# livesense-inc/fanlin-rs

Measured on AMD Instinct MI355X. Metric: images/sec whole-node (1080p→300×200 resize+encode); p50 per-image ms, higher is better.
Workload: dtype u8 (exact, as f16 subnormals) x the reference's f32 weights as three f16 terms -> f32 sums (vertical, v_mfma_f32_16x16x32_f16); 24-bit fixed-point intermediate (2^-14 steps, three i8 planes) x 24-bit fixed-point weights (2^-24 steps, three i8 digits), eight of the nine digit products -> exact i32 (h

## Files before the change

### fanlin-rs_amd/csrc/fl_batch.cpp

```cpp
#include <stdio.h>
#include <stdlib.h>

#include <algorithm>
#include <cassert>
#include <memory>
#include <optional>

#include "fl_context.h"

using namespace fl;

namespace {


enum Stage1Kind { S1_NONE = 0, S1_PLACE = 1, S1_GENERIC = 2, S1_STREAM = 3, S1_NEAREST = 4, S1_MFMA = 5, S1_TILE = 6, S1_WTILE = 7 };
constexpr size_t kNoScratch = ~(size_t)0;

struct Work {
    flgpu_plan plan;
    const flgpu_params *p;
    uint32_t cs, pre, sw, sh;
    Stage1Kind s1;
    const uint8_t *src;
    uint8_t *s1_dst = nullptr;
// ... 155 lines not shown
            if (!R) uniform = false;
            else {
                for (uint32_t r = 0; r < R; ++r)
                    for (uint32_t t = 0; t < T; ++t) {
                        const auto &v = by_job[jobs_in_order[r * T + t]];
                        for (uint32_t s2 = 0; s2 < S; ++s2) per_wg[triples[t][s2]].push_back(v[s2]);
                    }
                const uint32_t Lp = P - R * T;
                if (Lp) {
                    const uint32_t nt = (uint32_t)plan->tiles.size();
                    const uint32_t nb = std::max(1u, std::min(nt, (2u * G + Lp * S - 1u) / (Lp * S)));
                    const std::vector<MfmaItem> &bands = plan->items_for(nb);
                    std::vector<MfmaItem> units;
                    for (uint32_t p2 = R * T; p2 < P; ++p2)
                        for (MfmaItem u : bands) { u.job = jobs_in_order[p2]; units.push_back(u); }
                    std::stable_sort(units.begin(), units.end(), [](const MfmaItem &x, const MfmaItem &y) { return x.kb1 - x.kb0 > y.kb1 - y.kb0; });
                    std::vector<uint64_t> load(G, 0);
                    for (uint32_t b = 0; b < G; ++b) for (const MfmaItem &a : per_wg[b]) load[b] += a.kb1 - a.kb0;
                    for (const MfmaItem &u : units) {
                        uint32_t best = 0;
                        for (uint32_t b = 1; b < G; ++b) if (load[b] < load[best]) best = b;
                        per_wg[best].push_back(u);
                        load[best] += u.kb1 - u.kb0 + 2u;
                    }
                }
            }
        }
    }
    if (!uniform) { for (auto &v : per_wg) v.clear(); classic(); }
    std::vector<MfmaItem> flat;
    lists.assign(2u * G, 0u);
    for (uint32_t b = 0; b < G; ++b) {
        lists[2 * b] = (uint32_t)flat.size();
        lists[2 * b + 1] = (uint32_t)per_wg[b].size();
        flat.insert(flat.end(), per_wg[b].begin(), per_wg[b].end());
    }
    mitems.resize(base);
    mitems.insert(mitems.end(), flat.begin(), flat.end());
    nitems = (uint32_t)flat.size();
}

void fill_job(const Work &w, Job &j)
{
    memset(&j, 0, sizeof(j));
    const flgpu_plan &pl = w.plan;
    j.src = w.src;
    j.dst = w.s1_dst;
    j.src_bytes = w.sw * w.sh * w.cs;
    j.sw = w.sw; j.sh = w.sh;
    j.rw = pl.resized_w; j.rh = pl.resized_h;
    j.cx = pl.crop_x; j.cy = pl.crop_y;
    if (pl.letterboxed) {
        j.cw = std::min(pl.resized_w - pl.crop_x, pl.out_w - pl.place_x);
        j.ch = std::min(pl.resized_h - pl.crop_y, pl.out_h - pl.place_y);
    } else {
        j.cw = pl.out_w; j.ch = pl.out_h;
    }
    j.dw = pl.out_w; j.dh = pl.out_h;
    j.ox = pl.place_x; j.oy = pl.place_y;
    if (w.luma_mid) { j.dw = j.cw; j.dh = j.ch; j.ox = 0; j.oy = 0; }
    j.fill = (uint32_t)w.p->fill_r | ((uint32_t)w.p->fill_g << 8) | ((uint32_t)w.p->fill_b << 16) | (255u << 24);
    j.vtab = w.vtab; j.htab = w.htab;
    j.pad1 = w.tile_w;
    j.pad0 = w.tile_vplan;
    if (w.s1 == S1_NEAREST) {
        const float ry = (float)w.sh / (float)pl.resized_h, rx = (float)w.sw / (float)pl.resized_w;
        memcpy(&j.vtab, &ry, 4); memcpy(&j.htab, &rx, 4);
    }
}


uint32_t tile_width_for(const HostAxis &h, const HostAxis &v, uint32_t cx, uint32_t cw, uint32_t cy, uint32_t ch, uint32_t mc)
{
    for (uint32_t y0 = cy; y0 < cy + ch; y0 += 8u) {
        const uint32_t y1 = std::min(y0 + 8u, cy + ch);
        if (v.left[y1 - 1] + v.count[y1 - 1] - v.left[y0] > kTileVRows) return 0;
    }
    const uint32_t nc_max = kTileLdsFloats / (8u * mc);
    for (uint32_t tw = 256; tw >= 16; tw >>= 1) {
        bool fits = true;
        for (uint32_t x0 = cx; x0 < cx + cw && fits; x0 += tw) {
            const uint32_t x1 = std::min(x0 + tw, cx + cw);
            if (h.left[x1 - 1] + h.count[x1 - 1] - h.left[x0] > nc_max) fits = false;
            if (h.woff[x1 - 1] + h.count[x1 - 1] - h.woff[x0] > kTileWeightFloats) fits = false;
        }
        if (fits) return tw;
    }
    return 0;
}

void build_tile_vplan(const HostAxis &v, uint32_t cy, uint32_t ch, std::vector<uint32_t> &blk)
{
    const uint32_t nb = (ch + 7u) / 8u;
    uint32_t stride = 1;
    for (uint32_t b = 0; b < nb; ++b) {
        const uint32_t y0 = cy + 8u * b, y1 = std::min(y0 + 8u, cy + ch);
        stride = std::max(stride, v.left[y1 - 1] + v.count[y1 - 1] - v.left[y0]);
    }
    TileVPlanHeader hd{nb, stride, (uint32_t)(sizeof(TileVPlanHeader) / 4), (uint32_t)(sizeof(TileVPlanHeader) / 4) + 2u * nb};
    blk.assign((size_t)hd.dense_off + (size_t)nb * stride * 8u, 0u);
    memcpy(blk.data(), &hd, sizeof(hd));
    for (uint32_t b = 0; b < nb; ++b) {
        const uint32_t y0 = cy + 8u * b, y1 = std::min(y0 + 8u, cy + ch);
        const uint32_t top = v.left[y0], rv = v.left[y1 - 1] + v.count[y1 - 1] - top;
        blk[hd.bands_off + 2u * b] = top;
        blk[hd.bands_off + 2u * b + 1u] = rv;
        float *dense = reinterpret_cast<float *>(blk.data() + hd.dense_off) + (size_t)b * stride * 8u;
        for (uint32_t oy = y0; oy < y1; ++oy)
            for (uint32_t k = 0; k < v.count[oy]; ++k) dense[(size_t)(v.left[oy] + k - top) * 8u + (oy - y0)] = v.weights[v.woff[oy] + k];
    }
}

template <class Item, class Len>
void xcd_interleave(Item *first, uint32_t nitems, Len len_of)
{
#ifdef FL_EXPERIMENT
    static const bool no_xcd_order = [] { const char *e = getenv("FLGPU_NO_XCD_ORDER"); return e && e[0] == '1'; }();
#else
    constexpr bool no_xcd_order = false;
#endif
    std::vector<Item> tmp;
    for (uint32_t a = 0; a < nitems && !no_xcd_order;) {
        uint32_t b = a;
        const uint32_t len = len_of(first[a]);
        while (b < nitems && len_of(first[b]) == len) ++b;
        for (uint32_t g0 = a; g0 < b;) {
            uint32_t g1 = g0, njob = 0, prev = 0xffffffffu, per = 0, cur = 0;
            bool uniform = true;
            while (g1 < b) {
                if (first[g1].job != prev) {
                    if (njob == 8) break;
                    if (njob >= 1) { if (per == 0) per = cur; else if (cur != per) uniform = false; }
                    ++njob; prev = first[g1].job; cur = 0;
                }
                ++cur; ++g1;
            }
            if (per == 0) per = cur; else if (cur != per) uniform = false;
            if (uniform && njob > 1 && per > 1) {
                tmp.assign(first + g0, first + g1);
                for (uint32_t s2 = 0; s2 < per; ++s2)
                    for (uint32_t j2 = 0; j2 < njob; ++j2) first[g0 + s2 * njob + j2] = tmp[j2 * per + s2];
            }
            g0 = g1;
        }
        a = b;
    }
}



int jpeg_scratch(const flgpu_plan &pl, ScratchSizes &s)
{
    if (pl.out_w > 65535u || pl.out_h > 65535u) return FLGPU_ERR_UNSUPPORTED;
    const size_t units = (size_t)(pl.plane_w / 8u) * (pl.plane_h / 8u) * 3u;
    if (units * kJpegMaxUnitBytes * 8 >= ((size_t)1 << 32)) return FLGPU_ERR_UNSUPPORTED;
    s.jpeg_coef += align_up(units * sizeof(JpegUnit), 256);
    s.jpeg_off += align_up((units + 1) * sizeof(uint32_t), 256);
    s.jpeg_raw += align_up(units * kAcWordsPerUnit * sizeof(uint32_t), 256);
    return FLGPU_OK;
}

int png_scratch(const flgpu_plan &pl, ScratchSizes &s)
{
    const uint64_t fb = png_filtered_bytes(pl.out_w, pl.out_h, pl.out_c);
    if ((uint64_t)s.png_rows + pl.out_h >= (1ull << 31) || (uint64_t)s.png_segs + png_segments(fb) >= (1ull << 31)) return FLGPU_ERR_UNSUPPORTED;
    s.png_filt += align_up(fb, 256);
    s.png_rows += pl.out_h;
    s.png_segs += (uint32_t)png_segments(fb);
    return FLGPU_OK;
}

int webpll_scratch(const flgpu_plan &pl, ScratchSizes &s)
{
    const uint64_t npix = (uint64_t)pl.out_w * pl.out_h;
    if ((uint64_t)s.wll_tiles + webpll_tiles(npix) >= (1ull << 31) || webpll_max_out_bytes(pl.out_w, pl.out_h) / 4u >= (1ull << 32))
        return FLGPU_ERR_UNSUPPORTED;
    s.wll_res += align_up(npix * 4u, 256);
    s.wll_tok += align_up(npix * 2u, 256);
    s.wll_stream += align_up(webpll_max_out_bytes(pl.out_w, pl.out_h), 256);
    s.wll_tiles += (uint32_t)webpll_tiles(npix);
    s.wll_pics++;
    return FLGPU_OK;
}

bool vp8_fe_lf(uint32_t fe) { return fe >= FLGPU_FE_WEBP_LOSSY_LF && fe <= FLGPU_FE_WEBP_LOSSY_I4_AP_LF; }
bool vp8_fe_i4(uint32_t fe) { return fe == FLGPU_FE_WEBP_LOSSY_I4 || fe == FLGPU_FE_WEBP_LOSSY_I4_AP || fe == FLGPU_FE_WEBP_LOSSY_I4_LF || fe == FLGPU_FE_WEBP_LOSSY_I4_AP_LF; }
bool vp8_fe_ap(uint32_t fe) { return fe == FLGPU_FE_WEBP_LOSSY_AP || fe == FLGPU_FE_WEBP_LOSSY_I4_AP || fe == FLGPU_FE_WEBP_LOSSY_AP_LF || fe == FLGPU_FE_WEBP_LOSSY_I4_AP_LF; }
bool vp8_fe(uint32_t fe) { return fe == FLGPU_FE_WEBP_LOSSY || vp8_fe_i4(fe) || vp8_fe_ap(fe) || vp8_fe_lf(fe); }
int vp8_scratch(const flgpu_plan &pl, ScratchSizes &s, uint32_t fe)
{
    const bool i4 = vp8_fe_i4(fe), ap = vp8_fe_ap(fe);
    const bool fits = ap ? (i4 ? vp8_i4_ap_fits(pl.out_w, pl.out_h) : vp8_ap_fits(pl.out_w, pl.out_h)) : i4 ? vp8_i4_fits(pl.out_w, pl.out_h) : vp8_fits(pl.out_w, pl.out_h);
    if (!fits) return FLGPU_ERR_UNSUPPORTED;
    const uint64_t mbs = (uint64_t)vp8_mbs(pl.out_w) * vp8_mbs(pl.out_h);
    if (i4) s.vp8_i4_mbs += mbs;
    if (ap) s.vp8_ap_pics++;
    if (vp8_fe_lf(fe)) s.vp8_lf += vp8_lf_bytes(vp8_mbs(pl.out_w), vp8_mbs(pl.out_h));
    s.vp8_planes += align_up(vp8_planes_bytes(pl.out_w, pl.out_h), 256);
    s.vp8_rec += align_up(vp8_rec_bytes(vp8_mbs(pl.out_w), vp8_mbs(pl.out_h)), 256);
    s.vp8_mbs += mbs;
    s.vp8_pics++;
    return FLGPU_OK;
}

int plan_pictures(Batch &B, const flgpu_image *srcs, const flgpu_params *ps, bool same_params)
{
    for (size_t i = 0; i < B.n; ++i) {
        Work &w = B.work[i];
        const flgpu_image &s = srcs[i];
        w.p = same_params ? &ps[0] : &ps[i];
        if (!s.data || !B.dsts[i].data) return FLGPU_ERR_INVALID_ARG;
        int rc = flgpu_plan_output(w.p, s.width, s.height, s.channels, &w.plan);
        if (rc) return rc;
        if (s.capacity < (uint64_t)s.width * s.height * s.channels) return FLGPU_ERR_INVALID_ARG;
        if (B.dsts[i].capacity < w.plan.out_bytes) return FLGPU_ERR_BUFFER_TOO_SMALL;
        w.cs = s.channels; w.sw = w.plan.src_w; w.sh = w.plan.src_h;
        w.raw_w = s.width; w.raw_h = s.height;
        w.orient = w.p->orientation >= 2 ? w.p->orientation : 0;
        if (w.orient) { w.orient_off = B.scratch.o; B.scratch.o += align_up((size_t)s.width * s.height * s.channels, 256); }
        w.pre = w.p->grayscale ? PRE_GRAY : (w.p->inverse ? PRE_INVERT : PRE_NONE);
        w.src = s.data;
        w.final_dst = B.dsts[i].data;
        const flgpu_plan &pl = w.plan;
        const bool cropped = pl.crop_x || pl.crop_y || pl.out_w != pl.resized_w || pl.out_h != pl.resized_h;
        const bool pre_changes = (w.pre == PRE_INVERT) || (w.pre == PRE_GRAY && w.cs >= 3);
        if (!pre_changes) w.pre = PRE_NONE;
        if (pl.resampled) w.s1 = w.p->filter == FLGPU_FILTER_NEAREST ? S1_NEAREST : S1_GENERIC;
        else if (pre_changes || pl.letterboxed || cropped) w.s1 = S1_PLACE;
        else w.s1 = S1_NONE;
        const bool mfma_candidate = !B.dbg.on(DBG_NO_MFMA) && !B.dbg.on(DBG_FORCE_GENERIC) && (size_t)w.sw * w.cs >= 64u && (uint64_t)w.sh >= 2u * (uint64_t)pl.resized_h;
        if (pl.resampled && w.s1 == S1_GENERIC && !pre_changes && !w.orient && mfma_candidate && ((size_t)w.sw * w.cs) % 16u == 0 && (uintptr_t)s.data % 16u != 0) {
            w.align_off = B.scratch.al;
            B.scratch.al += align_up((size_t)s.width * s.height * s.channels, 256);
        }
        const bool blur = w.p->blur_sigma > 0.0f;
        const bool fe = w.p->front_end != FLGPU_FE_NONE;
        if (w.s1 != S1_NONE && !blur && !fe) w.s1_dst = w.final_dst;
        else if (w.s1 != S1_NONE) { w.s1_off = B.scratch.a; B.scratch.a += align_up(pl.pixel_bytes, 256); }
        if (blur && !fe) w.blur_dst = w.final_dst;
        else if (blur) { w.blur_off = B.scratch.b; B.scratch.b += align_up(pl.pixel_bytes, 256); }
        if (w.p->front_end == FLGPU_FE_JPEG) rc = jpeg_scratch(pl, B.scratch);
        if (w.p->front_end == FLGPU_FE_PNG) rc = png_scratch(pl, B.scratch);
        if (w.p->front_end == FLGPU_FE_WEBP_LOSSLESS) rc = webpll_scratch(pl, B.scratch);
        if (vp8_fe(w.p->front_end)) rc = vp8_scratch(pl, B.scratch, w.p->front_end);
        if (rc) return rc;
    }
    return FLGPU_OK;
}

int reserve_scratch(flgpu_ctx *c, Batch &B, hipStream_t st)
{
    const ScratchSizes &sz = B.scratch;
    FL_HIP(c, c->d_jpeg_coef.reserve(sz.jpeg_coef), "JPEG coefficient scratch");
    FL_HIP(c, c->d_jpeg_off.reserve(sz.jpeg_off), "JPEG offset scratch");
    FL_HIP(c, c->d_jpeg_raw.reserve(sz.jpeg_raw), "JPEG bit-stream scratch");
    FL_HIP(c, c->d_png_filt.reserve(sz.png_filt), "PNG filtered-row scratch");
    FL_HIP(c, c->d_png_chunks.reserve((size_t)sz.png_segs * kPngSegOutBytes), "PNG chunk scratch");
    FL_HIP(c, c->d_png_syms.reserve((size_t)sz.png_segs * kPngSegBytes * sizeof(uint16_t)), "PNG symbol scratch");
    FL_HIP(c, c->d_png_recs.reserve((size_t)sz.png_segs * 4u * sizeof(uint32_t)), "PNG segment records");
    FL_HIP(c, c->d_webpll_res.reserve(sz.wll_res), "WebP residual scratch");
    FL_HIP(c, c->d_webpll_tok.reserve(sz.wll_tok), "WebP token scratch");
    FL_HIP(c, c->d_webpll_tiles.reserve((size_t)sz.wll_tiles * sizeof(WebpllTile)), "WebP tile records");
    FL_HIP(c, c->d_webpll_pic.reserve((size_t)sz.wll_pics * kWebpllPicWords * sizeof(uint32_t)), "WebP per-picture scratch");
    FL_HIP(c, c->d_webpll_stream.reserve(sz.wll_stream), "WebP bit-stream scratch");
    FL_HIP(c, c->d_vp8_planes.reserve(sz.vp8_planes), "lossy WebP plane scratch");
    FL_HIP(c, c->d_vp8_rec.reserve(sz.vp8_rec), "lossy WebP reconstruction scratch");
    FL_HIP(c, c->d_vp8_lev.reserve(sz.vp8_mbs * kVp8MbLevels * sizeof(int16_t)), "lossy WebP level scratch");
    FL_HIP(c, c->d_vp8_info.reserve(sz.vp8_mbs * sizeof(uint32_t)), "lossy WebP macroblock records");
    FL_HIP(c, c->d_vp8_bm.reserve(sz.vp8_i4_mbs * 2u * sizeof(uint32_t)), "lossy WebP sub-block mode records");
    FL_HIP(c, c->d_vp8_tab.reserve((size_t)sz.vp8_ap_pics * kVp8TabBytes), "lossy WebP probability tables");
    FL_HIP(c, c->d_vp8_lf.reserve(sz.vp8_lf), "lossy WebP loop filter scratch");
    FL_HIP(c, c->d_vp8_sizes.reserve((size_t)sz.vp8_pics * kVp8SizeWords * sizeof(uint32_t)), "lossy WebP partition sizes");
    FL_HIP(c, c->d_tmp_o.reserve(sz.o), "orientation scratch");
    FL_HIP(c, c->d_tmp_al.reserve(sz.al), "alignment scratch");
    for (auto &w : B.work)
        if (w.align_off != kNoScratch) {
            uint8_t *al = static_cast<uint8_t *>(c->d_tmp_al.p) + w.align_off;
            FL_HIP(c, hipMemcpyAsync(al, w.src, (size_t)w.sw * w.sh * w.cs, hipMemcpyDeviceToDevice, st), "alignment copy");
            w.src = al;
        }
    FL_HIP(c, c->d_tmp_a.reserve(sz.a), "scratch A");
    FL_HIP(c, c->d_tmp_b.reserve(sz.b), "scratch B");
    for (auto &w : B.work) {
        if (w.orient) { w.raw_src = w.src; w.src = static_cast<uint8_t *>(c->d_tmp_o.p) + w.orient_off; }
        if (w.s1 == S1_NONE) w.s1_dst = const_cast<uint8_t *>(w.src);
        if (w.s1_off != kNoScratch) w.s1_dst = static_cast<uint8_t *>(c->d_tmp_a.p) + w.s1_off;
        if (w.blur_off != kNoScratch) w.blur_dst = static_cast<uint8_t *>(c->d_tmp_b.p) + w.blur_off;
    }
    return FLGPU_OK;
}


bool arena_nearly_full(const flgpu_ctx *c) { return c->h_arena.size() >= c->arena_cap_words - 1024; }

template <class Map, class Build> uint32_t cached_block(flgpu_ctx *c, Map &cache, const typename Map::key_type &key, Build &&build)
{
    auto it = cache.find(key);
    if (it != cache.end()) return it->second;
    std::vector<uint32_t> blk;
    build(blk);
    const uint32_t off = arena_append(c, blk.data(), blk.size());
    if (off) cache.emplace(key, off);
    return off;
}

bool try_wtile(flgpu_ctx *c, Work &w, const Job &j)
{
    WtPlan *wp = get_wtile_plan(c, w.vk, *w.va, w.hk, *w.ha, j.cx, j.cy, j.cw, j.ch, w.cs);
// ... 779 lines not shown
```

### fanlin-rs_amd/csrc/fl_jpeg.h

```cpp
#pragma once
#include <hip/hip_runtime.h>
#include <stdint.h>

namespace fl {

#define FL_JPEG_RESULT_OVERFLOW 4u
constexpr uint32_t kAcWordsPerUnit = 52;
constexpr uint32_t kUnitAcWords = 3;
struct alignas(16) JpegUnit {
    uint32_t meta;
    uint32_t ac[kUnitAcWords];
};
struct alignas(16) JpegJob {
    const uint8_t *src;
    uint8_t *dst;
    JpegUnit *units;
    uint32_t *unit_off;
    uint32_t *acbits;
    uint32_t *result;
    uint32_t w, h, c;
    uint32_t bx, by;
    uint32_t tab_off;
    uint32_t pad0;
    uint32_t dst_cap;
};

hipError_t launch_jpeg_encode(const JpegJob *jobs, const uint32_t *arena, uint32_t job_base, uint32_t njobs, uint32_t max_blocks,
                              hipStream_t st);

}
```

### fanlin-rs_amd/csrc/fl_jpeg.hip

```cpp
#include <hip/hip_runtime.h>
#include <stdint.h>

#include "fl_jpeg.h"
#include "fl_jpeg_tables.h"
#include "fl_pixel.h"
#include "fl_types.h"

namespace fl {

namespace {


constexpr int32_t F_0_298 = 2446, F_0_390 = 3196, F_0_541 = 4433, F_0_765 = 6270, F_0_899 = 7373, F_1_175 = 9633, F_1_501 = 12299,
                  F_1_847 = 15137, F_1_961 = 16069, F_2_053 = 16819, F_2_562 = 20995, F_3_072 = 25172;

struct Mat8 { int32_t a[8][8]; };

constexpr void fdct_linear(const int32_t in[8], int32_t out[8])
{
    int32_t t0 = in[0] + in[7], t1 = in[1] + in[6], t2 = in[2] + in[5], t3 = in[3] + in[4];
    const int32_t t10 = t0 + t3, t11 = t1 + t2;
    int32_t t12 = t0 - t3, t13 = t1 - t2;
    t0 = in[0] - in[7]; t1 = in[1] - in[6]; t2 = in[2] - in[5]; t3 = in[3] - in[4];
    out[0] = t10 + t11;
    out[4] = t10 - t11;
    int32_t z1 = (t12 + t13) * F_0_541;
    out[2] = z1 + t12 * F_0_765;
    out[6] = z1 - t13 * F_1_847;
    t12 = t0 + t2;
    t13 = t1 + t3;
    z1 = (t12 + t13) * F_1_175;
    t12 = t12 * (-F_0_390) + z1;
    t13 = t13 * (-F_1_961) + z1;
    z1 = (t0 + t3) * (-F_0_899);
    out[1] = t0 * F_1_501 + z1 + t12;
    out[7] = t3 * F_0_298 + z1 + t13;
    z1 = (t1 + t2) * (-F_2_562);
    out[3] = t1 * F_3_072 + z1 + t13;
    out[5] = t2 * F_2_053 + z1 + t12;
}

constexpr Mat8 make_fdct_matrix()
{
    Mat8 m{};
    for (int j = 0; j < 8; ++j) {
        int32_t e[8] = {0, 0, 0, 0, 0, 0, 0, 0}, o[8] = {0, 0, 0, 0, 0, 0, 0, 0};
        e[j] = 1;
        fdct_linear(e, o);
        for (int k = 0; k < 8; ++k) m.a[k][j] = o[k];
    }
    return m;
}

__constant__ Mat8 kFdct = make_fdct_matrix();

constexpr bool fdct_matrix_fits_i16()
{
    const Mat8 m = make_fdct_matrix();
    for (int k = 0; k < 8; ++k)
        for (int j = 0; j < 8; ++j)
            if (m.a[k][j] > 32767 || m.a[k][j] < -32768) return false;
    return true;
}
static_assert(fdct_matrix_fits_i16(), "the passes use v_dot2_i32_i16: matrix entries must be 16-bit");

typedef short i16x2 __attribute__((ext_vector_type(2)));
__device__ __forceinline__ i16x2 as_i16x2(uint32_t v) { return __builtin_bit_cast(i16x2, v); }
__device__ __forceinline__ uint32_t pack_i16(int32_t lo, int32_t hi) { return ((uint32_t)lo & 0xffffu) | ((uint32_t)hi << 16); }
__device__ __forceinline__ int32_t dot8_i16(const uint32_t m[4], const uint4 v)
{
    int32_t p = __builtin_amdgcn_sdot2(as_i16x2(m[0]), as_i16x2(v.x), 0, false);
    p = __builtin_amdgcn_sdot2(as_i16x2(m[1]), as_i16x2(v.y), p, false);
    p = __builtin_amdgcn_sdot2(as_i16x2(m[2]), as_i16x2(v.z), p, false);
    return __builtin_amdgcn_sdot2(as_i16x2(m[3]), as_i16x2(v.w), p, false);
}

struct NaturalOrder { uint8_t n[64]; };
constexpr NaturalOrder make_natural()
{
    NaturalOrder t{};
    for (int k = 0; k < 64; ++k) t.n[k] = kUnzigzag[k];
    return t;
}
__constant__ NaturalOrder kNatural = make_natural();

struct HuffLut { uint32_t e[256]; };

constexpr HuffLut make_lut(const HuffSpec &s)
{
    HuffLut t{};
    uint32_t code = 0;
    int k = 0;
    for (int l = 1; l <= 16; ++l) {
        for (int i = 0; i < s.len[l - 1]; ++i, ++k) t.e[s.val[k]] = ((uint32_t)l << 16) | code++;
        code <<= 1;
    }
    return t;
}

struct HuffAll { HuffLut ac[2], dc[2]; };
constexpr HuffAll make_all() { return HuffAll{{make_lut(kAcLuma), make_lut(kAcChroma)}, {make_lut(kDcLuma), make_lut(kDcChroma)}}; }
__constant__ HuffAll kHuff = make_all();


template <int N>
__device__ __forceinline__ uint32_t dpp_row_shr(uint32_t v)
{
    return (uint32_t)__builtin_amdgcn_update_dpp(0, (int)v, 0x110 + N, 0xf, 0xf, false);
}

__device__ __forceinline__ uint32_t wave_inclusive_scan(uint32_t v, uint32_t lane)
{
    (void)lane;
    v += dpp_row_shr<1>(v);
    v += dpp_row_shr<2>(v);
    v += dpp_row_shr<4>(v);
    v += dpp_row_shr<8>(v);
    v += (uint32_t)__builtin_amdgcn_update_dpp(0, (int)v, 0x142, 0xa, 0xf, false);
    v += (uint32_t)__builtin_amdgcn_update_dpp(0, (int)v, 0x143, 0xc, 0xf, false);
    return v;
}

__device__ __forceinline__ void wave_lds_sync()
{
    __builtin_amdgcn_fence(__ATOMIC_SEQ_CST, "wavefront");
    __builtin_amdgcn_wave_barrier();
}

constexpr uint32_t kPackThreads = 512;
constexpr uint32_t kPackWaves = kPackThreads / 64;

__device__ __forceinline__ uint32_t wg_exclusive_scan(uint32_t v, uint32_t *s_w, uint32_t *total)
{
    const uint32_t lane = threadIdx.x & 63u, wave = threadIdx.x >> 6;
    const uint32_t inc = wave_inclusive_scan(v, lane);
    __syncthreads();
    if (lane == 63u) s_w[wave] = inc;
    __syncthreads();
    uint32_t base = 0, sum = 0;
#pragma unroll
    for (uint32_t i = 0; i < kPackWaves; ++i) { const uint32_t t = s_w[i]; if (i < wave) base += t; sum += t; }
    *total = sum;
    return base + inc - v;
}

__device__ __forceinline__ uint32_t coef_size(int32_t v)
{
    const uint32_t mag = (uint32_t)(v < 0 ? -v : v);
    return mag ? 32u - (uint32_t)__clz(mag) : 0u;
}


#ifndef FL_JPEG_BPW
#define FL_JPEG_BPW 16
#define FL_JPEG_WPG 2
#define FL_JPEG_PREFETCH 3
#endif
constexpr uint32_t kBlocksPerWave = FL_JPEG_BPW;
constexpr uint32_t kWavesPerWg = FL_JPEG_WPG;
constexpr uint32_t kPrefetch = FL_JPEG_PREFETCH;
static_assert(kBlocksPerWave == 32u || kBlocksPerWave == 16u, "the coding phase's lane mapping");
constexpr uint32_t kJpegThreads = 64u * kWavesPerWg;
constexpr uint32_t kBlocksPerWg = kWavesPerWg * kBlocksPerWave;
constexpr uint32_t kUnitsPerWave = 3u * kBlocksPerWave;

static_assert(63u * (16u + 10u) <= kAcWordsPerUnit * 32u, "a unit's AC code must fit its acbits slot");

struct WaveLds {
    int16_t coef[kUnitsPerWave][64];
    uint64_t nz[kUnitsPerWave];
    __attribute__((aligned(16))) int16_t smp[3][64];
    __attribute__((aligned(16))) int16_t p1[3][64];
};

__device__ __forceinline__ void stage_ac_luts(uint32_t *s_ac)
{
    for (uint32_t i = threadIdx.x; i < 512u; i += kJpegThreads) s_ac[i] = kHuff.ac[i >> 8].e[i & 255u];
    __syncthreads();
}

template <bool kRgba>
__device__ __forceinline__ uint32_t block_pixel(const JpegJob &jb, uint32_t brow, uint32_t bcol, uint32_t r, uint32_t c)
{
    uint32_t px = bcol * 8u + c, py = brow * 8u + r;
    px = px < jb.w ? px : jb.w - 1u;
    py = py < jb.h ? py : jb.h - 1u;
    if constexpr (kRgba) return ((const __attribute__((address_space(1))) uint32_t *)jb.src)[(size_t)py * jb.w + px];
    uint32_t pr, pg, pb, pa;
    load_rgba(jb.src + ((size_t)py * jb.w + px) * jb.c, jb.c, pr, pg, pb, pa);
    return pr | (pg << 8) | (pb << 16);
}

__device__ __forceinline__ void dct_quant_block(const uint32_t (&smp)[3], uint32_t nat, uint32_t r, uint32_t c, const uint32_t (&m1)[4],
                                                const uint32_t (&m2)[4], uint4 k1, const uint32_t (&q)[3], const uint32_t (&magic)[3],
                                                WaveLds &w, int32_t (&qv)[3])
{
#pragma unroll
    for (int k = 0; k < 3; ++k) w.smp[k][nat] = (int16_t)smp[k];
    wave_lds_sync();
#pragma unroll
    for (int k = 0; k < 3; ++k) {
        const int32_t p = dot8_i16(m1, *reinterpret_cast<const uint4 *>(w.smp[k] + r * 8));
        const int32_t v1 = ((p << k1.x) + (int32_t)k1.y) >> 11;
        w.p1[k][c * 8 + r] = (int16_t)v1;
    }
    wave_lds_sync();
#pragma unroll
    for (int k = 0; k < 3; ++k) {
        const int32_t p2 = dot8_i16(m2, *reinterpret_cast<const uint4 *>(w.p1[k] + c * 8));
        const int32_t d = (p2 + (int32_t)k1.z) >> k1.w;
        const int32_t sg = d >> 31;
        const uint32_t an = (uint32_t)((d ^ sg) - sg) >> 3;
        const uint32_t rq = __umulhi(2u * an + q[k], magic[k]);
        qv[k] = ((int32_t)rq ^ sg) - sg;
    }
}

typedef __attribute__((address_space(1))) uint32_t global_u32;
typedef uint32_t u32x4 __attribute__((ext_vector_type(4)));
typedef __attribute__((address_space(1))) u32x4 global_u32x4;
static_assert(sizeof(JpegUnit) == sizeof(u32x4) && kUnitAcWords == 3u, "a unit's record is one 16-byte access");

struct UnitBits {
    uint64_t acc;
    uint32_t pend, total, wi;
    global_u32 *out;
    uint32_t w0, w1, w2;
    __device__ __forceinline__ void word(uint32_t v)
    {
        w0 = wi == 0u ? v : w0;
        w1 = wi == 1u ? v : w1;
        w2 = wi == 2u ? v : w2;
        if (wi >= kUnitAcWords) out[wi] = v;
        ++wi;
    }
    __device__ __forceinline__ void put(uint32_t code, uint32_t len)
    {
        acc = (acc << len) | code;
        pend += len;
        total += len;
        if (pend >= 32u) { pend -= 32u; word((uint32_t)(acc >> pend)); }
    }
};

template <bool kRgba>
__device__ __forceinline__ void transform_blocks(const JpegJob &jb, const uint32_t *__restrict__ arena, uint32_t first, uint32_t count,
                                                 uint32_t lane, WaveLds &w)
{
    const uint32_t nat = kNatural.n[lane], r = nat >> 3, c = nat & 7u;
    uint32_t m1[4], m2[4];
#pragma unroll
    for (int j = 0; j < 4; ++j) {
        m1[j] = pack_i16(kFdct.a[c][2 * j], kFdct.a[c][2 * j + 1]);
        m2[j] = pack_i16(kFdct.a[r][2 * j], kFdct.a[r][2 * j + 1]);
    }
    const uint8_t *qt = reinterpret_cast<const uint8_t *>(arena + jb.tab_off) + 624;
    const uint32_t *mg = reinterpret_cast<const uint32_t *>(qt + 128);
    const uint32_t q[3] = {qt[nat], qt[64 + nat], qt[64 + nat]};
    const uint32_t magic[3] = {mg[nat], mg[64 + nat], mg[64 + nat]};
    const uint4 k1 = {(c == 0u || c == 4u) ? 13u : 0u, c == 0u ? (uint32_t)(-(8 * 128) * 8192) : (c == 4u ? 0u : 1u << 10),
                      (r == 0u || r == 4u) ? 2u : 1u << 14, (r == 0u || r == 4u) ? 2u : 15u};
    uint32_t brow = first / jb.bx, bcol = first - brow * jb.bx;
    uint32_t ahead[kPrefetch];
#pragma unroll
    for (uint32_t j = 0; j < kPrefetch; ++j) {
        ahead[j] = block_pixel<kRgba>(jb, brow, bcol, r, c);
        if (++bcol == jb.bx) { bcol = 0; ++brow; }
    }
    for (uint32_t i = 0; i < count; ++i) {
        const uint32_t rgb = kRgba ? ahead[0] & 0xffffffu : ahead[0];
#pragma unroll
        for (uint32_t j = 0; j + 1u < kPrefetch; ++j) ahead[j] = ahead[j + 1u];
        ahead[kPrefetch - 1u] = block_pixel<kRgba>(jb, brow, bcol, r, c);
        if (++bcol == jb.bx) { bcol = 0; ++brow; }
        uint32_t smp[3];
        jfif_px(rgb, smp[0], smp[1], smp[2]);
        const bool flat = __ballot(rgb != (uint32_t)__builtin_amdgcn_readfirstlane((int)rgb)) == 0ull;
        if (flat) {
            if (lane == 0u) {
#pragma unroll
                for (int k = 0; k < 3; ++k) {
                    const int32_t d = 64 * ((int32_t)smp[k] - 128);
                    const int32_t sg = d >> 31;
                    const uint32_t an = (uint32_t)((d ^ sg) - sg) >> 3;
                    const uint32_t rq = __umulhi(2u * an + q[k], magic[k]);
                    w.coef[i * 3u + k][0] = (int16_t)(((int32_t)rq ^ sg) - sg);
                    w.nz[i * 3u + k] = 0ull;
                }
            }
            continue;
        }
        int32_t qv[3];
        dct_quant_block(smp, nat, r, c, m1, m2, k1, q, magic, w, qv);
#pragma unroll
        for (int k = 0; k < 3; ++k) {
            w.coef[i * 3u + k][lane] = (int16_t)qv[k];
            const uint64_t nz = __ballot(qv[k] != 0) & ~1ull;
            if (lane == 0u) w.nz[i * 3u + k] = nz;
        }
    }
}

__global__ __launch_bounds__(kJpegThreads) void jpeg_dct_quant_kernel(const JpegJob *__restrict__ jobs, const uint32_t *__restrict__ arena,
                                                                      uint32_t job_base)
{
    __shared__ WaveLds s_w[kWavesPerWg];
    __shared__ uint32_t s_ac[512];
    const JpegJob jb = jobs[job_base + blockIdx.y];
    const uint32_t wave = threadIdx.x >> 6, lane = threadIdx.x & 63u;
    const uint32_t nblocks = jb.bx * jb.by;
    if (blockIdx.x * kBlocksPerWg >= nblocks) return;
    stage_ac_luts(s_ac);
    const uint32_t first = blockIdx.x * kBlocksPerWg + wave * kBlocksPerWave;
    if (first >= nblocks) return;
    const uint32_t count = min(kBlocksPerWave, nblocks - first);
    WaveLds &w = s_w[wave];

    if (jb.c == 4u && (reinterpret_cast<uintptr_t>(jb.src) & 3u) == 0u) transform_blocks<true>(jb, arena, first, count, lane, w);
    else transform_blocks<false>(jb, arena, first, count, lane, w);
    wave_lds_sync();

    uint32_t b, u, u_end;
    bool chroma;
    if constexpr (kBlocksPerWave == 32u) {
        b = lane & 31u;
        chroma = lane >= 32u;
        u = b * 3u + (chroma ? 1u : 0u);
        u_end = b * 3u + (chroma ? 3u : 1u);
    } else {
        b = lane & 15u;
        chroma = lane >= 16u;
        u = b * 3u + (lane >> 4);
        u_end = lane >= 48u ? u : u + 1u;
    }
    if (b >= count) return;
    const uint32_t *tab = s_ac + (chroma ? 256u : 0u);
    const uint32_t eob = tab[0], zrl = tab[0xF0];
    for (; u < u_end; ++u) {
        const uint32_t unit = first * 3u + u;
        const int16_t *cf = w.coef[u];
        uint64_t m = w.nz[u];
        UnitBits ub{0ull, 0u, 0u, 0u, (global_u32 *)jb.acbits + (size_t)unit * kAcWordsPerUnit, 0u, 0u, 0u};
        uint32_t prev = 0;
        uint32_t pos = (uint32_t)__builtin_ctzll(m | (1ull << 63));
        int32_t v = cf[pos];
        while (m) {
            const uint32_t cpos = pos;
            const int32_t cv = v;
            m &= m - 1ull;
            pos = (uint32_t)__builtin_ctzll(m | (1ull << 63));
            v = cf[pos];
            uint32_t run = cpos - prev - 1u;
            prev = cpos;
            while (run > 15u) { ub.put(zrl & 0xffffu, zrl >> 16); run -= 16u; }
            const uint32_t mag = (uint32_t)(cv < 0 ? -cv : cv);
            const uint32_t size = 32u - (uint32_t)__clz(mag);
            const uint32_t value = (uint32_t)(cv + (cv >> 31)) & ((1u << size) - 1u);
            const uint32_t e = tab[(run << 4) | size];
            ub.put(((e & 0xffffu) << size) | value, (e >> 16) + size);
        }
        if (prev != 63u) ub.put(eob & 0xffffu, eob >> 16);
        if (ub.pend) ub.word((uint32_t)(ub.acc << (32u - ub.pend)));
        const u32x4 rec = {((uint32_t)(uint16_t)cf[0]) | (ub.total << 16), ub.w0, ub.w1, ub.w2};
        ((global_u32x4 *)jb.units)[unit] = rec;
    }
}


constexpr uint32_t kWinWords = 8192;

__device__ __forceinline__ void win_or(uint32_t *win, uint32_t wbase, uint64_t g, uint32_t val)
{
    const uint64_t W = g >> 5;
    const uint32_t sh = (uint32_t)g & 31u;
    const uint32_t hi = val >> sh, lo = sh ? val << (32u - sh) : 0u;
    if (hi && W >= wbase && W < (uint64_t)wbase + kWinWords) atomicOr(&win[W - wbase], hi);
    if (lo && W + 1 >= wbase && W + 1 < (uint64_t)wbase + kWinWords) atomicOr(&win[W + 1 - wbase], lo);
}

constexpr uint32_t kDcCodes = 12;

__device__ __forceinline__ uint32_t dc_code(const uint32_t *s_dc, uint32_t u, uint32_t meta, uint32_t prev_meta, uint32_t *len)
{
    const int32_t dc = (int16_t)(meta & 0xffffu), prev = (int16_t)(prev_meta & 0xffffu);
    const int32_t diff = dc - prev;
    const uint32_t size = coef_size(diff);
    const uint32_t value = (uint32_t)(diff < 0 ? diff - 1 : diff) & ((1u << size) - 1u);
    const uint32_t e = s_dc[((u % 3u) ? kDcCodes : 0u) + size];
    *len = (e >> 16) + size;
    return (((e & 0xffffu) << size) | value) << (32u - *len);
}

struct PackUnit { u32x4 rec; uint32_t prev; };
__device__ __forceinline__ PackUnit load_pack_unit(const JpegJob &jb, uint32_t u, uint32_t u_end)
{
    const global_u32x4 *recs = (const global_u32x4 *)jb.units;
    const uint32_t uc = min(u, u_end - 1u);
    PackUnit p;
    p.rec = recs[uc];
    p.prev = ((const global_u32 *)(recs + (max(uc, 3u) - 3u)))[0];
    return p;
}
__device__ __forceinline__ PackUnit take_pack_unit(PackUnit p, uint32_t u, uint32_t u_end)
{
    if (u >= u_end) p.rec = u32x4{0u, 0u, 0u, 0u};
    if (u < 3u || u >= u_end) p.prev = 0u;
    return p;
}

#ifndef FL_JPEG_PACK_DEPTH
#define FL_JPEG_PACK_DEPTH 1
#endif
constexpr uint32_t kPackDepth = FL_JPEG_PACK_DEPTH;

__global__ __launch_bounds__(kPackThreads) void jpeg_pack_kernel(const JpegJob *__restrict__ jobs, const uint32_t *__restrict__ arena,
                                                                 uint32_t job_base)
{
    __shared__ uint32_t s_win[kWinWords];
    __shared__ uint32_t s_w[kPackWaves], s_carry, s_lo, s_hi, s_dc[2u * kDcCodes];
    const JpegJob jb = jobs[job_base + blockIdx.x];
    const uint32_t tid = threadIdx.x;
    const uint32_t nunits = jb.bx * jb.by * 3u;
    constexpr uint32_t T = kPackThreads;

    PackUnit ahead[kPackDepth];
#pragma unroll
    for (uint32_t j = 0; j < kPackDepth; ++j) ahead[j] = load_pack_unit(jb, j * T + tid, nunits);
    for (uint32_t i = tid; i < kWinWords; i += T) s_win[i] = 0u;
    if (tid < 2u * kDcCodes) s_dc[tid] = kHuff.dc[tid / kDcCodes].e[tid % kDcCodes];
    if (tid == 0u) s_carry = 0u;
    __syncthreads();
    for (uint32_t base0 = 0; base0 < nunits; base0 += kPackDepth * T) {
#pragma unroll
        for (uint32_t j = 0; j < kPackDepth; ++j) {
            const uint32_t base = base0 + j * T;
            if (base >= nunits) break;
            const uint32_t u = base + tid;
            const PackUnit next = load_pack_unit(jb, u + kPackDepth * T, nunits);
            const PackUnit cur = take_pack_unit(ahead[j], u, nunits);
            ahead[j] = next;
            const uint32_t m = cur.rec.x;
            const uint32_t nw = ((m >> 16) + 31u) >> 5;
            uint32_t len = 0, dl = 0, dcw = 0;
            if (u < nunits) {
                dcw = dc_code(s_dc, u, m, cur.prev, &dl);
                len = dl + (m >> 16);
            }
            uint32_t chunk;
            const uint32_t ex = wg_exclusive_scan(len, s_w, &chunk);
            const uint32_t carry = s_carry;
            if (u < nunits) {
                const uint32_t off = carry + ex;
                ((global_u32 *)jb.unit_off)[u] = off;
                win_or(s_win, 0u, off, dcw);
                win_or(s_win, 0u, (uint64_t)off + dl, cur.rec.y);
                win_or(s_win, 0u, (uint64_t)off + dl + 32u, cur.rec.z);
                win_or(s_win, 0u, (uint64_t)off + dl + 64u, cur.rec.w);
                for (uint32_t w = kUnitAcWords; w < nw; ++w)
                    win_or(s_win, 0u, (uint64_t)off + dl + 32u * w, ((const global_u32 *)jb.acbits)[(size_t)u * kAcWordsPerUnit + w]);
            }
            __syncthreads();
            if (tid == 0u) s_carry = carry + chunk;
            __syncthreads();
        }
    }
    const uint32_t total_bits = s_carry;
    if (tid == 0u) jb.unit_off[nunits] = total_bits;
    __threadfence_block();
    __syncthreads();
    const uint32_t nbytes = (total_bits + 7u) >> 3, limit = jb.dst_cap;
    const uint8_t *hdr = reinterpret_cast<const uint8_t *>(arena + jb.tab_off);
    for (uint32_t i = tid; i < kJpegHeaderBytes; i += T) if (i < limit) jb.dst[i] = hdr[i];

    uint32_t ff_before = 0;
    for (uint32_t wbase = 0; wbase * 32ull < total_bits; wbase += kWinWords) {
        const uint64_t wb = (uint64_t)wbase * 32u, we = wb + (uint64_t)kWinWords * 32u;
        if (wbase != 0u) {
            for (uint32_t i = tid; i < kWinWords; i += T) s_win[i] = 0u;
            if (tid == 0u) {
                uint32_t lo = 0, hi = nunits;
                while (lo < hi) { const uint32_t mid = (lo + hi) >> 1; if (jb.unit_off[mid + 1u] > wb) hi = mid; else lo = mid + 1u; }
                s_lo = lo;
                uint32_t lo2 = lo, hi2 = nunits;
                while (lo2 < hi2) { const uint32_t mid = (lo2 + hi2) >> 1; if (jb.unit_off[mid] >= we) hi2 = mid; else lo2 = mid + 1u; }
                s_hi = lo2;
            }
        } else if (tid == 0u) { s_lo = 0u; s_hi = 0u; }
        __syncthreads();
        const uint32_t u_lo = s_lo, u_hi = s_hi;
        for (uint32_t ub = u_lo; ub < u_hi; ub += T / 2u) {
            const uint32_t u = ub + (tid >> 1), j = tid & 1u;
            if (u < u_hi) {
                const PackUnit p = take_pack_unit(load_pack_unit(jb, u, u_hi), u, u_hi);
                const uint32_t m = p.rec.x, off = jb.unit_off[u];
                uint32_t dl;
                const uint32_t dcw = dc_code(s_dc, u, m, p.prev, &dl);
                if (j == 0u) win_or(s_win, wbase, off, dcw);
                const uint32_t nw = ((m >> 16) + 31u) >> 5;
                win_or(s_win, wbase, (uint64_t)off + dl + 32u * j, j ? p.rec.z : p.rec.y);
                if (j == 0u) win_or(s_win, wbase, (uint64_t)off + dl + 64u, p.rec.w);
                for (uint32_t w = j ? 3u : 4u; w < nw; w += 2u)
                    win_or(s_win, wbase, (uint64_t)off + dl + 32u * w, ((const global_u32 *)jb.acbits)[(size_t)u * kAcWordsPerUnit + w]);
            }
        }
        __syncthreads();
        if (tid == 0u && (total_bits & 7u) && (total_bits >> 5) >= wbase && (total_bits >> 5) < wbase + kWinWords)
            s_win[(total_bits >> 5) - wbase] |= (0xFFu >> (total_bits & 7u)) << (24u - 8u * ((total_bits >> 3) & 3u));
        __syncthreads();
        const uint32_t win_bytes = (uint32_t)min((uint64_t)kWinWords * 4u, (uint64_t)nbytes - (uint64_t)wbase * 4u);
        if (tid == 0u) s_carry = 0u;
        __syncthreads();
        for (uint32_t base = 0; base < win_bytes; base += 4u * T) {
            const uint32_t i = base + tid * 4u;
            const uint32_t word = i < win_bytes ? s_win[i >> 2] : 0u;
            const uint32_t valid = i < win_bytes ? (win_bytes - i < 4u ? win_bytes - i : 4u) : 0u;
            uint32_t ff = 0;
#pragma unroll
            for (uint32_t k = 0; k < 4; ++k) ff += (k < valid && ((word >> (24u - 8u * k)) & 255u) == 255u) ? 1u : 0u;
            uint32_t chunk;
            const uint32_t ex = wg_exclusive_scan(ff, s_w, &chunk);
            const uint32_t carry = s_carry;
            uint64_t o = (uint64_t)kJpegHeaderBytes + (uint64_t)wbase * 4u + i + ff_before + carry + ex;
#pragma unroll
            for (uint32_t k = 0; k < 4; ++k) {
                if (k < valid) {
                    const uint32_t b = (word >> (24u - 8u * k)) & 255u;
                    if (o < limit) jb.dst[o] = (uint8_t)b;
                    ++o;
                    if (b == 255u) { if (o < limit) jb.dst[o] = 0u; ++o; }
                }
            }
            __syncthreads();
            if (tid == 0u) s_carry = carry + chunk;
            __syncthreads();
        }
        ff_before += s_carry;
        __syncthreads();
    }
    if (tid == 0u) {
        const uint64_t end = (uint64_t)kJpegHeaderBytes + nbytes + ff_before;
        if (end + 2u <= limit) {
            jb.dst[end] = 0xFF; jb.dst[end + 1u] = 0xD9;
            jb.result[1] = (uint32_t)(end + 2u);
        } else {
            jb.result[1] = 0u;
            atomicOr(&jb.result[0], FL_JPEG_RESULT_OVERFLOW);
        }
    }
}

}

hipError_t launch_jpeg_encode(const JpegJob *jobs, const uint32_t *arena, uint32_t job_base, uint32_t njobs, uint32_t max_blocks,
                              hipStream_t st)
{
    if (!njobs || !max_blocks) return hipSuccess;
    hipLaunchKernelGGL(jpeg_dct_quant_kernel, dim3((max_blocks + kBlocksPerWg - 1) / kBlocksPerWg, njobs), dim3(kJpegThreads), 0, st, jobs, arena, job_base);
    FL_LAUNCH_CHECK();
    hipLaunchKernelGGL(jpeg_pack_kernel, dim3(njobs), dim3(kPackThreads), 0, st, jobs, arena, job_base);
    FL_LAUNCH_CHECK();
    return hipSuccess;
}

}
```

Baseline: 590,000.

## Split luma AC coding into two records per block to balance lanes

The JPEG entropy-coding phase now emits four records per 8x8 block: Y split into a low-frequency part (AC positions 1..10) and a high part, plus Cb and Cr. With 16 blocks per wave, each of the 64 lanes codes exactly one record. Previously lanes 48-63 sat idle while luma lanes carried the heaviest work, so this evens out the divergent Huffman loop. The pack kernel and DC coding are adjusted so the Y-high record carries no DC code. The cost is a third more records to write, scan and pack, and slightly more scratch memory.

```diff
diff --git a/fanlin-rs_amd/csrc/fl_batch.cpp b/fanlin-rs_amd/csrc/fl_batch.cpp
--- a/fanlin-rs_amd/csrc/fl_batch.cpp
+++ b/fanlin-rs_amd/csrc/fl_batch.cpp
@@ -331,8 +331,9 @@
 int jpeg_scratch(const flgpu_plan &pl, ScratchSizes &s)
 {
     if (pl.out_w > 65535u || pl.out_h > 65535u) return FLGPU_ERR_UNSUPPORTED;
-    const size_t units = (size_t)(pl.plane_w / 8u) * (pl.plane_h / 8u) * 3u;
-    if (units * kJpegMaxUnitBytes * 8 >= ((size_t)1 << 32)) return FLGPU_ERR_UNSUPPORTED;
+    const size_t blocks = (size_t)(pl.plane_w / 8u) * (pl.plane_h / 8u);
+    if (blocks * 3u * kJpegMaxUnitBytes * 8 >= ((size_t)1 << 32)) return FLGPU_ERR_UNSUPPORTED;
+    const size_t units = blocks * kUnitsPerBlock;
     s.jpeg_coef += align_up(units * sizeof(JpegUnit), 256);
     s.jpeg_off += align_up((units + 1) * sizeof(uint32_t), 256);
     s.jpeg_raw += align_up(units * kAcWordsPerUnit * sizeof(uint32_t), 256);
diff --git a/fanlin-rs_amd/csrc/fl_jpeg.h b/fanlin-rs_amd/csrc/fl_jpeg.h
--- a/fanlin-rs_amd/csrc/fl_jpeg.h
+++ b/fanlin-rs_amd/csrc/fl_jpeg.h
@@ -7,6 +7,7 @@
 #define FL_JPEG_RESULT_OVERFLOW 4u
 constexpr uint32_t kAcWordsPerUnit = 52;
 constexpr uint32_t kUnitAcWords = 3;
+constexpr uint32_t kUnitsPerBlock = 4;
 struct alignas(16) JpegUnit {
     uint32_t meta;
     uint32_t ac[kUnitAcWords];
diff --git a/fanlin-rs_amd/csrc/fl_jpeg.hip b/fanlin-rs_amd/csrc/fl_jpeg.hip
--- a/fanlin-rs_amd/csrc/fl_jpeg.hip
+++ b/fanlin-rs_amd/csrc/fl_jpeg.hip
@@ -151,15 +151,13 @@
 }
 
 
-#ifndef FL_JPEG_BPW
-#define FL_JPEG_BPW 16
-#define FL_JPEG_WPG 2
-#define FL_JPEG_PREFETCH 3
-#endif
-constexpr uint32_t kBlocksPerWave = FL_JPEG_BPW;
-constexpr uint32_t kWavesPerWg = FL_JPEG_WPG;
-constexpr uint32_t kPrefetch = FL_JPEG_PREFETCH;
-static_assert(kBlocksPerWave == 32u || kBlocksPerWave == 16u, "the coding phase's lane mapping");
+constexpr uint32_t kBlocksPerWave = 16;
+constexpr uint32_t kWavesPerWg = 2;
+constexpr uint32_t kPrefetch = 3;
+constexpr uint32_t kLumaCut = 10;
+constexpr uint32_t kLumaLowMask = (2u << kLumaCut) - 2u;
+static_assert(kLumaCut >= 1u && kLumaCut <= 30u, "the lower part's mask is taken from the low word of the unit's mask");
+static_assert(kUnitsPerBlock == 4u, "records per block: Y-low, Y-high, Cb, Cr");
 constexpr uint32_t kJpegThreads = 64u * kWavesPerWg;
 constexpr uint32_t kBlocksPerWg = kWavesPerWg * kBlocksPerWave;
 constexpr uint32_t kUnitsPerWave = 3u * kBlocksPerWave;
@@ -320,50 +318,40 @@
     else transform_blocks<false>(jb, arena, first, count, lane, w);
     wave_lds_sync();
 
-    uint32_t b, u, u_end;
-    bool chroma;
-    if constexpr (kBlocksPerWave == 32u) {
-        b = lane & 31u;
-        chroma = lane >= 32u;
-        u = b * 3u + (chroma ? 1u : 0u);
-        u_end = b * 3u + (chroma ? 3u : 1u);
-    } else {
-        b = lane & 15u;
-        chroma = lane >= 16u;
-        u = b * 3u + (lane >> 4);
-        u_end = lane >= 48u ? u : u + 1u;
-    }
+    const uint32_t b = lane & 15u, part = lane >> 4;
     if (b >= count) return;
-    const uint32_t *tab = s_ac + (chroma ? 256u : 0u);
+    const bool upper = part == 3u;
+    const uint32_t u = b * 3u + (upper ? 0u : part);
+    const uint32_t rec = (first + b) * kUnitsPerBlock + (part == 0u ? 0u : upper ? 1u : part + 1u);
+    const uint32_t *tab = s_ac + ((part == 1u || part == 2u) ? 256u : 0u);
     const uint32_t eob = tab[0], zrl = tab[0xF0];
-    for (; u < u_end; ++u) {
-        const uint32_t unit = first * 3u + u;
-        const int16_t *cf = w.coef[u];
-        uint64_t m = w.nz[u];
-        UnitBits ub{0ull, 0u, 0u, 0u, (global_u32 *)jb.acbits + (size_t)unit * kAcWordsPerUnit, 0u, 0u, 0u};
-        uint32_t prev = 0;
-        uint32_t pos = (uint32_t)__builtin_ctzll(m | (1ull << 63));
-        int32_t v = cf[pos];
-        while (m) {
-            const uint32_t cpos = pos;
-            const int32_t cv = v;
-            m &= m - 1ull;
-            pos = (uint32_t)__builtin_ctzll(m | (1ull << 63));
-            v = cf[pos];
-            uint32_t run = cpos - prev - 1u;
-            prev = cpos;
-            while (run > 15u) { ub.put(zrl & 0xffffu, zrl >> 16); run -= 16u; }
-            const uint32_t mag = (uint32_t)(cv < 0 ? -cv : cv);
-            const uint32_t size = 32u - (uint32_t)__clz(mag);
-            const uint32_t value = (uint32_t)(cv + (cv >> 31)) & ((1u << size) - 1u);
-            const uint32_t e = tab[(run << 4) | size];
-            ub.put(((e & 0xffffu) << size) | value, (e >> 16) + size);
-        }
-        if (prev != 63u) ub.put(eob & 0xffffu, eob >> 16);
-        if (ub.pend) ub.word((uint32_t)(ub.acc << (32u - ub.pend)));
-        const u32x4 rec = {((uint32_t)(uint16_t)cf[0]) | (ub.total << 16), ub.w0, ub.w1, ub.w2};
-        ((global_u32x4 *)jb.units)[unit] = rec;
-    }
+    const int16_t *cf = w.coef[u];
+    const uint64_t all = w.nz[u];
+    const uint32_t lower = (uint32_t)all & kLumaLowMask;
+    uint64_t m = part == 0u ? (uint64_t)lower : upper ? all & ~(uint64_t)kLumaLowMask : all;
+    UnitBits ub{0ull, 0u, 0u, 0u, (global_u32 *)jb.acbits + (size_t)rec * kAcWordsPerUnit, 0u, 0u, 0u};
+    uint32_t prev = upper ? 31u - (uint32_t)__clz(lower | 1u) : 0u;
+    uint32_t pos = (uint32_t)__builtin_ctzll(m | (1ull << 63));
+    int32_t v = cf[pos];
+    while (m) {
+        const uint32_t cpos = pos;
+        const int32_t cv = v;
+        m &= m - 1ull;
+        pos = (uint32_t)__builtin_ctzll(m | (1ull << 63));
+        v = cf[pos];
+        uint32_t run = cpos - prev - 1u;
+        prev = cpos;
+        while (run > 15u) { ub.put(zrl & 0xffffu, zrl >> 16); run -= 16u; }
+        const uint32_t mag = (uint32_t)(cv < 0 ? -cv : cv);
+        const uint32_t size = 32u - (uint32_t)__clz(mag);
+        const uint32_t value = (uint32_t)(cv + (cv >> 31)) & ((1u << size) - 1u);
+        const uint32_t e = tab[(run << 4) | size];
+        ub.put(((e & 0xffffu) << size) | value, (e >> 16) + size);
+    }
+    if (part != 0u && prev != 63u) ub.put(eob & 0xffffu, eob >> 16);
+    if (ub.pend) ub.word((uint32_t)(ub.acc << (32u - ub.pend)));
+    const u32x4 out = {(upper ? 0u : (uint32_t)(uint16_t)cf[0]) | (ub.total << 16), ub.w0, ub.w1, ub.w2};
+    ((global_u32x4 *)jb.units)[rec] = out;
 }
 
 
@@ -382,13 +370,15 @@
 
 __device__ __forceinline__ uint32_t dc_code(const uint32_t *s_dc, uint32_t u, uint32_t meta, uint32_t prev_meta, uint32_t *len)
 {
+    const uint32_t slot = u & 3u;
     const int32_t dc = (int16_t)(meta & 0xffffu), prev = (int16_t)(prev_meta & 0xffffu);
     const int32_t diff = dc - prev;
     const uint32_t size = coef_size(diff);
     const uint32_t value = (uint32_t)(diff < 0 ? diff - 1 : diff) & ((1u << size) - 1u);
-    const uint32_t e = s_dc[((u % 3u) ? kDcCodes : 0u) + size];
-    *len = (e >> 16) + size;
-    return (((e & 0xffffu) << size) | value) << (32u - *len);
+    const uint32_t e = s_dc[(slot >= 2u ? kDcCodes : 0u) + size];
+    const uint32_t l = (e >> 16) + size;
+    *len = slot == 1u ? 0u : l;
+    return slot == 1u ? 0u : (((e & 0xffffu) << size) | value) << (32u - l);
 }
 
 struct PackUnit { u32x4 rec; uint32_t prev; };
@@ -398,13 +388,13 @@
     const uint32_t uc = min(u, u_end - 1u);
     PackUnit p;
     p.rec = recs[uc];
-    p.prev = ((const global_u32 *)(recs + (max(uc, 3u) - 3u)))[0];
+    p.prev = ((const global_u32 *)(recs + (max(uc, kUnitsPerBlock) - kUnitsPerBlock)))[0];
     return p;
 }
 __device__ __forceinline__ PackUnit take_pack_unit(PackUnit p, uint32_t u, uint32_t u_end)
 {
     if (u >= u_end) p.rec = u32x4{0u, 0u, 0u, 0u};
-    if (u < 3u || u >= u_end) p.prev = 0u;
+    if (u < kUnitsPerBlock || u >= u_end) p.prev = 0u;
     return p;
 }
 
@@ -420,7 +410,7 @@
     __shared__ uint32_t s_w[kPackWaves], s_carry, s_lo, s_hi, s_dc[2u * kDcCodes];
     const JpegJob jb = jobs[job_base + blockIdx.x];
     const uint32_t tid = threadIdx.x;
-    const uint32_t nunits = jb.bx * jb.by * 3u;
+    const uint32_t nunits = jb.bx * jb.by * kUnitsPerBlock;
     constexpr uint32_t T = kPackThreads;
 
     PackUnit ahead[kPackDepth];
```

After: 551,600. 6.5% lower.
